# ywyue/AGILE3D

Hardware: AMD Instinct MI355X
Metric: scenes/s (80k-voxel, 10 clicks) (higher is better)
Workload: dtype f32; 1 GPU; batch of 16 synthetic 79736-voxel scenes, 10 clicks each (5 objects x 2), scene build + forward_backbone + 1 forward_mask per scene, fp32, eval; voxels=79736, queries=20, parallelism=scene-sharded x1 (no data-path collective), global_batch=16, steps_in_flight_per_gpu=4

## Files before the change

agile3d_amd/csrc/decoder.hip:

```cpp
#include "common.h"
#include <algorithm>
#include <type_traits>
#include <vector>

namespace a3d {

typedef float f32x4 __attribute__((ext_vector_type(4)));
#define A3D_GLOBAL __attribute__((address_space(1)))
template <typename T>
__device__ __forceinline__ T gld(const T* p) { return *(const T A3D_GLOBAL*)p; }
template <typename T>
__device__ __forceinline__ void gst(T* p, T v) { *(T A3D_GLOBAL*)p = v; }
__device__ __forceinline__ f32x4 gld4(const float* p) { return *(const f32x4 A3D_GLOBAL*)p; }
__device__ __forceinline__ void gst4(float* p, f32x4 v) { *(f32x4 A3D_GLOBAL*)p = v; }
__device__ __forceinline__ bool block_any(int pred, int* slot) {
  if (threadIdx.x == 0) *slot = 0;
  __syncthreads();
  if (pred) *slot = 1;
  __syncthreads();
  return *(volatile int*)slot != 0;
}
template <typename T>
__device__ __forceinline__ T gld_agent(const T* p) {
  return __hip_atomic_load((const T A3D_GLOBAL*)p, __ATOMIC_RELAXED, __HIP_MEMORY_SCOPE_AGENT);
// ... 255 lines not shown
        const bool blocked = pr >= n || (qmask[qt] && lab != obj[qt]);
        s[t] = blocked ? kNegBig : s[t];
        mx = fmaxf(mx, s[t]);
      }
      mx = rows_max(mx);
      const float mnew = fmaxf(m[qt], mx);
      const float sc = exp2_fast(m[qt] - mnew);
      m[qt] = mnew;
      f32x4 p;
      float ps = 0.f;
#pragma unroll
      for (int t = 0; t < 4; ++t) {
        p[t] = exp2_fast(s[t] - mnew);
        ps += p[t];
      }
      l[qt] = l[qt] * sc + ps;
      acc[qt] *= sc;
#pragma unroll
      for (int t = 0; t < 4; ++t) acc[qt] = __builtin_amdgcn_mfma_f32_16x16x4f32(vf[t], p[t], acc[qt], 0, 0, 0);
    }
  }
#pragma unroll
  for (int qt = 0; qt < QT; ++qt) {
    if (qt >= nqt) break;
    float lt = l[qt];
    lt = rows_sum(lt);
    float* pq = part + (((size_t)h * qp_total + qb0 + qt * 16 + j) * nchunk + chunk) * kPartStride;
    if (g == 0) {
      pq[0] = m[qt];
      pq[1] = lt;
    }
#pragma unroll
    for (int t = 0; t < 4; ++t) pq[2 + 4 * g + t] = acc[qt][t];
  }
}

template <int QT>
__global__ void __launch_bounds__(512) k_c2s_attn(const float* __restrict__ Kc, const float* __restrict__ V,
                                                  int n, const float* qproj, const int* qobj,
                                                  const unsigned char* labels, const int* counts,
                                                  float* part, int qp_total) {
  c2s_attn_body<QT>(Kc, V, n, qproj, qobj, labels, counts, part, qp_total, (int)blockIdx.y * (QT * 16), QT, (int)blockIdx.x,
                    (int)gridDim.x);
}
template <int QT>
__global__ void __launch_bounds__(512) k_c2s_attn_b(const DecSampleDev* __restrict__ samples) {
  const DecSampleDev& sm = samples[blockIdx.y];
  const int nchunk = (sm.n + kC2SChunk - 1) / kC2SChunk;
  if ((int)blockIdx.x >= nchunk) return;
  c2s_attn_body<QT>(sm.k0, sm.v0, sm.n, sm.qproj, sm.qobj, nullptr, nullptr, sm.part, sm.qp, 0, min(sm.nqt, QT), (int)blockIdx.x, nchunk);
}


template <int QT>
__global__ void __launch_bounds__(512) k_kv_c2s(const DecSampleDev* __restrict__ samples, int ns, int layer,
                                                const float* __restrict__ Wk, const float* __restrict__ Wv,
                                                const float* __restrict__ bk, const float* __restrict__ bv) {
  extern __shared__ __attribute__((aligned(16))) char smem[];
  constexpr int QP = QT * 16;
  constexpr int HW = QT <= 2 ? 4 : 2, WPG = H / HW, SPW = 8 / WPG;
  constexpr bool SWZ = QT == 4;
  constexpr int LDQ = SWZ ? 128 : 132;
  const DecSampleDev& sm = sample_of_wg(samples, ns);
  const int lb = blockIdx.x - sm.wg_begin, nwg = sm.wg_end - sm.wg_begin;
  const int n = sm.n, ngroups = (n + 15) / 16, qp_total = QP;
  const float* __restrict__ X = layer_input(sm, layer);
  const float* __restrict__ Pe = sm.posenc;
  const float* qproj = sm.qproj;
  const int* qobj = sm.qobj;
  const unsigned char* labels = layer > 0 ? sm.labels : nullptr;
  const int* counts = layer > 0 ? sm.counts + (size_t)(layer - 1) * (A3D_MAX_QUERIES + 1) : nullptr;
  float* part = sm.part;
  f32x4* Wkl = (f32x4*)smem;
  f32x4* Wvl = Wkl + 8 * 8 * 64;
  float* qp_l = (float*)(Wvl + 8 * 8 * 64);
  float* bk_l = qp_l + QP * LDQ;
  float* bv_l = bk_l + D;
  const int lane = threadIdx.x & 63, wave = threadIdx.x >> 6;
  const int g = lane >> 4, j = lane & 15;
  const int slot = lb * SPW + wave / WPG, nslots = nwg * SPW;
  f32x4 xs[8], pe[8];
  unsigned lab_nx = 0u;
  if (slot < ngroups) {
    const size_t row = (size_t)min(slot * 16 + j, n - 1);
    if (labels) lab_nx = gld((const unsigned*)(labels + slot * 16 + 4 * g));
#pragma unroll
    for (int S = 0; S < 8; ++S) xs[S] = gld4(X + row * D + 16 * S + 4 * g);
#pragma unroll
    for (int S = 0; S < 8; ++S) pe[S] = gld4(Pe + row * D + 16 * S + 4 * g);
  }
  {
    constexpr int TOT = 2 * 8 * 8 * 64;
    for (int base = threadIdx.x; base < TOT; base += 8 * 512) {
      f32x4 t8[8];
#pragma unroll
      for (int u = 0; u < 8; ++u) {
        const int e = base + u * 512;
        if (e < TOT) t8[u] = e < TOT / 2 ? ((const f32x4*)Wk)[e] : ((const f32x4*)Wv)[e - TOT / 2];
      }
#pragma unroll
      for (int u = 0; u < 8; ++u)
        if (base + u * 512 < TOT) Wkl[base + u * 512] = t8[u];
    }
  }
  for (int e = threadIdx.x; e < QP * 32; e += 512) {
    const int r = e >> 5, c = e & 31;
    *(f32x4*)(qp_l + r * LDQ + (SWZ ? (c ^ (r & 15)) : c) * 4) = gld4(qproj + (size_t)r * D + c * 4);
  }
  if (!SWZ && threadIdx.x < D) {
    bk_l[threadIdx.x] = bk[threadIdx.x];
    bv_l[threadIdx.x] = bv[threadIdx.x];
  }
  int obj[QT];
  bool qmask[QT];
#pragma unroll
  for (int qt = 0; qt < QT; ++qt) {
    obj[qt] = gld(qobj + qt * 16 + j);
    qmask[qt] = labels != nullptr && obj[qt] >= 0 && gld(counts + obj[qt]) > 0;
  }
  __syncthreads();
  const int h0 = (wave % WPG) * HW;
  f32x4 bkr[HW];
  float bvr[HW];
#pragma unroll
  for (int hl = 0; hl < HW; ++hl) {
    bkr[hl] = (f32x4){0.f, 0.f, 0.f, 0.f};
    bvr[hl] = 0.f;
    if constexpr (SWZ) {
      bkr[hl] = *(const f32x4*)(bk + 16 * (h0 + hl) + 4 * g);
      bvr[hl] = bv[16 * (h0 + hl) + j];
    }
  }
  float m[HW][QT], l[HW][QT];
  f32x4 acc[HW][QT];
#pragma unroll
  for (int hl = 0; hl < HW; ++hl)
#pragma unroll
    for (int qt = 0; qt < QT; ++qt) {
      m[hl][qt] = kNegBig;
      l[hl][qt] = 0.f;
      acc[hl][qt] = (f32x4){0.f, 0.f, 0.f, 0.f};
    }
  for (int grp = slot; grp < ngroups; grp += nslots) {
    const int p0 = grp * 16;
    const unsigned lab4 = lab_nx;
    const int next = grp + nslots < ngroups ? grp + nslots : grp;
    const size_t nrow = (size_t)min(next * 16 + j, n - 1);
    if (labels) lab_nx = gld((const unsigned*)(labels + next * 16 + 4 * g));
    f32x4 kf[HW], vv[HW];
#pragma unroll
    for (int hl = 0; hl < HW; ++hl) {
      kf[hl] = SWZ ? bkr[hl] : *(const f32x4*)(bk_l + 16 * (h0 + hl) + 4 * g);
      const float bvj = SWZ ? bvr[hl] : bv_l[16 * (h0 + hl) + j];
      vv[hl] = (f32x4){bvj, bvj, bvj, bvj};
    }
    {
      f32x4 wk = Wkl[(0 * 8 + h0) * 64 + lane], wv = Wvl[(0 * 8 + h0) * 64 + lane];
#pragma unroll
      for (int S = 0; S < 8; ++S) {
        const f32x4 xp = xs[S] + pe[S];
#pragma unroll
        for (int hl = 0; hl < HW; ++hl) {
          const int i2 = S * HW + hl + 1, S2 = i2 / HW, hl2 = i2 % HW;
          f32x4 nk = wk, nv = wv;
          if (i2 < 8 * HW) {
            nk = Wkl[(S2 * 8 + h0 + hl2) * 64 + lane];
            nv = Wvl[(S2 * 8 + h0 + hl2) * 64 + lane];
          }
          __builtin_amdgcn_sched_barrier(0);
#pragma unroll
          for (int t = 0; t < 4; ++t) {
            kf[hl] = __builtin_amdgcn_mfma_f32_16x16x4f32(wk[t], xp[t], kf[hl], 0, 0, 0);
            vv[hl] = __builtin_amdgcn_mfma_f32_16x16x4f32(xs[S][t], wv[t], vv[hl], 0, 0, 0);
          }
          __builtin_amdgcn_sched_barrier(0);
          wk = nk;
          wv = nv;
        }
        xs[S] = gld4(X + nrow * D + 16 * S + 4 * g);
        pe[S] = gld4(Pe + nrow * D + 16 * S + 4 * g);
        __builtin_amdgcn_sched_barrier(0);
      }
    }
    auto qfrag = [&](int qt, int h) {
      const int c = 4 * h + g;
      return *(const f32x4*)(qp_l + (qt * 16 + j) * LDQ + (SWZ ? (c ^ j) : c) * 4);
    };
    f32x4 qf_n = qfrag(0, h0);
    f32x4 mb[QT];
#pragma unroll
    for (int qt = 0; qt < QT; ++qt)
#pragma unroll
      for (int t = 0; t < 4; ++t) {
        const int pr = p0 + 4 * g + t;
        const int lab = (int)((lab4 >> (8 * t)) & 0xffu);
        const bool blocked = pr >= n || (qmask[qt] && lab != obj[qt]);
        mb[qt][t] = blocked ? kNegBig : 0.f;
      }
#pragma unroll
    for (int hl = 0; hl < HW; ++hl) {
      const int h = h0 + hl;
#pragma unroll
      for (int qt = 0; qt < QT; ++qt) {
        const f32x4 qf = qf_n;
        {
          const int i2 = hl * QT + qt + 1;
          if (i2 < HW * QT) qf_n = qfrag(i2 % QT, h0 + i2 / QT);
        }
        f32x4 sc4 = mb[qt];
#pragma unroll
        for (int t = 0; t < 4; ++t) sc4 = __builtin_amdgcn_mfma_f32_16x16x4f32(kf[hl][t], qf[t], sc4, 0, 0, 0);
        float mx = kNegBig;
#pragma unroll
        for (int t = 0; t < 4; ++t) mx = fmaxf(mx, sc4[t]);
        mx = rows_max(mx);
        const float mnew = fmaxf(m[hl][qt], mx);
        const float scl = exp2_fast(m[hl][qt] - mnew);
        m[hl][qt] = mnew;
        f32x4 pw;
        float ps = 0.f;
#pragma unroll
        for (int t = 0; t < 4; ++t) {
          pw[t] = exp2_fast(sc4[t] - mnew);
          ps += pw[t];
        }
        l[hl][qt] = l[hl][qt] * scl + ps;
        acc[hl][qt] *= scl;
#pragma unroll
        for (int t = 0; t < 4; ++t) acc[hl][qt] = __builtin_amdgcn_mfma_f32_16x16x4f32(vv[hl][t], pw[t], acc[hl][qt], 0, 0, 0);
      }
    }
  }
  {
    constexpr int REC = 6 * 64;
    float* red = (float*)smem;
    const int sg = wave / WPG, wl = wave % WPG;
    __syncthreads();
    if (sg > 0) {
#pragma unroll
      for (int hl = 0; hl < HW; ++hl)
#pragma unroll
        for (int qt = 0; qt < QT; ++qt) {
          float* r = red + ((size_t)((sg - 1) * WPG + wl) * (HW * QT) + hl * QT + qt) * REC + lane;
          r[0] = m[hl][qt];
          r[64] = l[hl][qt];
#pragma unroll
          for (int t = 0; t < 4; ++t) r[128 + 64 * t] = acc[hl][qt][t];
        }
    }
    __syncthreads();
    if (sg > 0) return;
#pragma unroll
    for (int hl = 0; hl < HW; ++hl)
#pragma unroll
      for (int qt = 0; qt < QT; ++qt) {
        float mm = m[hl][qt], ll = l[hl][qt];
        f32x4 aa = acc[hl][qt];
#pragma unroll
        for (int o = 1; o < SPW; ++o) {
          const float* r = red + ((size_t)((o - 1) * WPG + wl) * (HW * QT) + hl * QT + qt) * REC + lane;
          const float mo = r[0];
          const float mnew = fmaxf(mm, mo);
          const float sa = exp2_fast(mm - mnew), sb = exp2_fast(mo - mnew);
          mm = mnew;
          ll = ll * sa + r[64] * sb;
#pragma unroll
          for (int t = 0; t < 4; ++t) aa[t] = aa[t] * sa + r[128 + 64 * t] * sb;
        }
        const int h = h0 + hl;
        const float lt = rows_sum(ll);
        float* pq = part + (((size_t)h * qp_total + qt * 16 + j) * nwg + lb) * kPartStride;
        if (g == 0) {
          gst(pq, mm);
          gst(pq + 1, lt);
        }
#pragma unroll
        for (int t = 0; t < 4; ++t) gst(pq + 2 + 4 * g + t, aa[t]);
      }
  }
}
constexpr int kFusedC2SGrid = 256;

__global__ void __launch_bounds__(64) k_c2s_combine(const QuerySample* __restrict__ qs, int cached0) {
  const QuerySample& smp = qs[blockIdx.y];
  const int QP = smp.qp;
  const int q = blockIdx.x / H, h = blockIdx.x % H, lane = threadIdx.x;
  if (q >= smp.meta->nq) return;
  const float* __restrict__ part = smp.part;
  const int nchunk = cached0 ? smp.n_part0 : smp.n_part;
  float* attn = smp.B.attn;
  float m = kNegBig, l = 0.f, o[DH];
#pragma unroll
  for (int d = 0; d < DH; ++d) o[d] = 0.f;
  for (int ch = lane; ch < nchunk; ch += 64) {
    const float* p = part + (((size_t)h * QP + q) * nchunk + ch) * kPartStride;
    const float pm = gld(p);
    const float mn = fmaxf(m, pm);
    const float a = exp2f(m - mn), b = exp2f(pm - mn);
    l = l * a + gld(p + 1) * b;
#pragma unroll
    for (int d = 0; d < DH; ++d) o[d] = o[d] * a + gld(p + 2 + d) * b;
    m = mn;
  }
  float M = m;
#pragma unroll
  for (int off = 32; off > 0; off >>= 1) M = fmaxf(M, __shfl_xor(M, off, 64));
  const float sc = exp2f(m - M);
  l *= sc;
#pragma unroll
  for (int off = 32; off > 0; off >>= 1) l += __shfl_xor(l, off, 64);
#pragma unroll
  for (int d = 0; d < DH; ++d) {
    float v = o[d] * sc;
#pragma unroll
    for (int off = 32; off > 0; off >>= 1) v += __shfl_xor(v, off, 64);
    if (lane == d) gst(attn + (size_t)q * D + h * DH + d, v / l);
  }
}

template <int QT>
__global__ void __launch_bounds__(512) k_s2c_attn_wide(const float* __restrict__ Qs, int n, const float* ks,
                                                       const float* vs, int nq, int nblk, float* O) {
  constexpr int QP = QT * 16, LD = 132;
  extern __shared__ __attribute__((aligned(16))) char smem[];
// ... 411 lines not shown
      const f32x4 be = *(const f32x4*)(be_l + 16 * ct + 4 * g);
#pragma unroll
      for (int t = 0; t < 4; ++t) y[ct][t] = (y[ct][t] - mean) * rstd * ga[t] + be[t];
      if (p0 + j < n) gst4(yrow + 16 * ct + 4 * g, y[ct]);
    }
#pragma unroll
    for (int qt = 0; qt < QT; ++qt) {
      f32x4 acc = (f32x4){0.f, 0.f, 0.f, 0.f};
#pragma unroll
      for (int S = 0; S < 8; ++S) {
        const f32x4 ef = *(const f32x4*)(E_l + (qt * 16 + j) * LD + 16 * S + 4 * g);
#pragma unroll
        for (int t = 0; t < 4; ++t) acc = __builtin_amdgcn_mfma_f32_16x16x4f32(y[S][t], ef[t], acc, 0, 0, 0);
      }
#pragma unroll
      for (int t = 0; t < 4; ++t) Lw[(4 * g + t) * LL + qt * 16 + j] = acc[t];
    }
    asm volatile("s_waitcnt lgkmcnt(0)" ::: "memory");
    for (int o = g; o <= K; o += 4) {
      const int qb = o == 0 ? n_fg : qr_l[o], qe = o == 0 ? nq : qr_l[o + 1];
      float mxv = -3.4e38f;
      for (int q = qb; q < qe; ++q) mxv = fmaxf(mxv, Lw[j * LL + q]);
      Ow[j * (K + 1) + o] = mxv;
    }
    asm volatile("s_waitcnt lgkmcnt(0)" ::: "memory");
    if (lane < 16 && p0 + lane < n) {
      float best = Ow[lane * (K + 1)];
      int bi = 0;
      for (int o = 1; o <= K; ++o) {
        const float v = Ow[lane * (K + 1) + o];
        if (v > best) {
          best = v;
          bi = o;
        }
      }
      gst(labels + p0 + lane, (unsigned char)bi);
      atomicAdd(&hist[bi], 1);
    }
    const int rows = min(16, n - p0);
    for (int e = lane; e < rows * (K + 1); e += 64) gst(logits + (size_t)p0 * (K + 1) + e, Ow[e]);
    asm volatile("s_waitcnt lgkmcnt(0)" ::: "memory");
    grp = next;
  }
  __syncthreads();
  for (int e = threadIdx.x; e <= K; e += 512)
    if (hist[e]) atomicAdd(&counts[e], hist[e]);
}

template <int QT, int NW, bool KG = false, bool QC = false>
__global__ void __launch_bounds__(NW * 64) k_s2c_out(const DecSampleDev* __restrict__ samples, int ns, int layer,
                                                 const float* __restrict__ Wq, const float* __restrict__ bq,
                                                 const float* __restrict__ Wo, const float* __restrict__ bo,
                                                 const float* __restrict__ gamma, const float* __restrict__ beta, int nqr_max,
                                                 int Kmax) {
  constexpr int LD = 136, NT = NW * 64;
  constexpr bool PF = NW == 8;
  const DecSampleDev& sm = sample_of_wg(samples, ns);
  const int lb = blockIdx.x - sm.wg_begin, nwg = sm.wg_end - sm.wg_begin;
  const int n = sm.n, ngroups = (n + 15) / 16, nq = sm.nq, n_fg = sm.n_fg, K = sm.K;
  const float* __restrict__ X = layer_input(sm, layer);
  const float* __restrict__ Pe = sm.posenc;
  float* __restrict__ Y = (layer & 1) ? sm.bufD : sm.bufC;
  float* logits = sm.logits + (size_t)layer * n * (K + 1);
  unsigned char* labels = sm.labels;
  int* counts = sm.counts + (size_t)layer * (A3D_MAX_QUERIES + 1);
  const int LT = nqr_max + 4;
  extern __shared__ __attribute__((aligned(16))) char smem[];
  f32x4* Wql = (f32x4*)smem;
  f32x4* Wol = Wql + 8 * 8 * 64;
  float* ks_l = (float*)(Wol + 8 * 8 * 64);
  float* vt_l = ks_l + (KG ? 0 : nqr_max * LD);
  float* bq_l = vt_l + D * LT;
  float* bo_l = bq_l + D;
  float* ga_l = bo_l + D;
  float* be_l = ga_l + D;
  float* O_l = be_l + D;
  int* hist = (int*)(O_l + NW * 16 * (Kmax + 1));
  int* qr_l = hist + Kmax + 1;
  float* sb_l = (float*)(qr_l + Kmax + 2);
  for (int e = threadIdx.x; e < QT * 16; e += NT) sb_l[e] = e < nq ? 0.f : kNegBig;
  for (int e = threadIdx.x; e <= K + 1; e += NT) qr_l[e] = gld(sm.qrange + e);
  for (int e = threadIdx.x; e <= K; e += NT) hist[e] = 0;
  if (threadIdx.x < D) {
    bq_l[threadIdx.x] = bq[threadIdx.x];
    bo_l[threadIdx.x] = bo[threadIdx.x];
    ga_l[threadIdx.x] = gamma[threadIdx.x];
    be_l[threadIdx.x] = beta[threadIdx.x];
  }
  {
    constexpr int TOT = 8 * 8 * 64;
    for (int base = threadIdx.x; base < TOT; base += 4 * NT) {
      f32x4 t8[8];
#pragma unroll
      for (int u = 0; u < 4; ++u)
        if (base + u * NT < TOT) {
          t8[u] = ((const f32x4*)Wq)[base + u * NT];
          t8[4 + u] = ((const f32x4*)Wo)[base + u * NT];
        }
#pragma unroll
      for (int u = 0; u < 4; ++u)
        if (base + u * NT < TOT) {
          Wql[base + u * NT] = t8[u];
          Wol[base + u * NT] = t8[4 + u];
        }
    }
  }
  for (int e = threadIdx.x; e < nqr_max * 32; e += NT) {
// ... 150 lines not shown
#pragma unroll
          for (int u = 0; u < 2; ++u) vf[u][kt] = lds4((u ? vt_a1 : vt_a) + kt * 64);
#pragma unroll
        for (int kt = 0; kt < QT; ++kt)
#pragma unroll
          for (int t = 0; t < 4; ++t)
#pragma unroll
            for (int u = 0; u < 2; ++u) acc[u] = __builtin_amdgcn_mfma_f32_16x16x4f32(vf[u][kt][t], sc[u][kt][t], acc[u], 0, 0, 0);
      }
#pragma unroll
      for (int u = 0; u < 2; ++u) acc[u] *= inv[u];
#pragma unroll
      for (int i = 0; i < 8; ++i) {
        const int u = i >> 2, ct = 2 * (i & 3);
        f32x4 n0 = wo0, n1 = wo1;
        if (i + 1 < 8) {
          const int u2 = (i + 1) >> 2, ct2 = 2 * ((i + 1) & 3);
          n0 = lds4(wo_a + (u2 * 512 + ct2 * 64) * 16);
          n1 = lds4(wo_a + (u2 * 512 + ct2 * 64 + 64) * 16);
        }
        __builtin_amdgcn_sched_barrier(0);
#pragma unroll
        for (int t = 0; t < 4; ++t) {
          y[ct] = __builtin_amdgcn_mfma_f32_16x16x4f32(wo0[t], acc[u][t], y[ct], 0, 0, 0);
          y[ct + 1] = __builtin_amdgcn_mfma_f32_16x16x4f32(wo1[t], acc[u][t], y[ct + 1], 0, 0, 0);
        }
        __builtin_amdgcn_sched_barrier(0);
        wo0 = n0;
        wo1 = n1;
      }
    }
    float sum = 0.f;
#pragma unroll
    for (int ct = 0; ct < 8; ++ct) sum += y[ct][0] + y[ct][1] + y[ct][2] + y[ct][3];
    sum = rows_sum(sum);
    const float mean = sum * (1.f / D);
    float var = 0.f;
#pragma unroll
    for (int ct = 0; ct < 8; ++ct)
#pragma unroll
      for (int t = 0; t < 4; ++t) {
        const float d = y[ct][t] - mean;
        var += d * d;
      }
    var = rows_sum(var);
    const float rstd = rsqrtf(var * (1.f / D) + kLnEps);
    float* yrow = Y + (size_t)prow * D;
#pragma unroll
    for (int ct = 0; ct < 8; ++ct) {
      const f32x4 ga = *(const f32x4*)(ga_l + 16 * ct + 4 * g);
      const f32x4 be = *(const f32x4*)(be_l + 16 * ct + 4 * g);
#pragma unroll
      for (int t = 0; t < 4; ++t) y[ct][t] = (y[ct][t] - mean) * rstd * ga[t] + be[t];
      if (p0 + j < n) gst4(yrow + 16 * ct + 4 * g, y[ct]);
    }
    f32x4 ef[QT][8];
#pragma unroll
    for (int qt = 0; qt < QT; ++qt) {
      const float* er = sm.E + (size_t)min(qt * 16 + j, nq - 1) * D + 4 * g;
#pragma unroll
      for (int S = 0; S < 8; ++S) ef[qt][S] = gld4(er + 16 * S);
    }
    f32x4 lg[QT], lg2[QT];
#pragma unroll
    for (int qt = 0; qt < QT; ++qt) lg[qt] = lg2[qt] = (f32x4){0.f, 0.f, 0.f, 0.f};
#pragma unroll
    for (int S = 0; S < 8; S += 2)
#pragma unroll
      for (int t = 0; t < 4; ++t)
#pragma unroll
        for (int qt = 0; qt < QT; ++qt) {
          lg[qt] = __builtin_amdgcn_mfma_f32_16x16x4f32(ef[qt][S][t], y[S][t], lg[qt], 0, 0, 0);
          lg2[qt] = __builtin_amdgcn_mfma_f32_16x16x4f32(ef[qt][S + 1][t], y[S + 1][t], lg2[qt], 0, 0, 0);
        }
#pragma unroll
    for (int qt = 0; qt < QT; ++qt) lg[qt] += lg2[qt];
    float best = 0.f;
    int bi = 0;
    for (int o = 0; o <= K; ++o) {
      float mxv = -3.4e38f;
#pragma unroll
      for (int qt = 0; qt < QT; ++qt)
#pragma unroll
        for (int t = 0; t < 4; ++t)
          if (((oidp[qt] >> (8 * t)) & 255u) == (unsigned)o) mxv = fmaxf(mxv, lg[qt][t]);
      mxv = rows_max(mxv);
      if (g == (o & 3)) Ow[j * (K + 1) + o] = mxv;
      if (o == 0 || mxv > best) {
        best = mxv;
        bi = o;
      }
    }
    if (g == 0 && p0 + j < n) {
      gst(labels + p0 + j, (unsigned char)bi);
      atomicAdd(&hist[bi], 1);
    }
    asm volatile("s_waitcnt lgkmcnt(0)" ::: "memory");
    const int rows = min(16, n - p0);
    for (int e = lane; e < rows * (K + 1); e += 64) gst(logits + (size_t)p0 * (K + 1) + e, Ow[e]);
    asm volatile("s_waitcnt lgkmcnt(0)" ::: "memory");
    grp = next;
  }
  __syncthreads();
  for (int e = threadIdx.x; e <= K; e += NT)
    if (hist[e]) atomicAdd(&counts[e], hist[e]);
}

struct QueryLayerW {
  const float *c2s_in_wt, *c2s_in_b, *c2s_out_wt, *c2s_out_b, *c2s_norm_w, *c2s_norm_b;
  const float *c2c_in_wt, *c2c_in_b, *c2c_out_wt, *c2c_out_b, *c2c_norm_w, *c2c_norm_b;
  const float *ffn_w1t, *ffn_b1, *ffn_w2t, *ffn_b2, *ffn_norm_w, *ffn_norm_b;
  const float *s2c_in_wt, *s2c_in_b;
  const float *dn_w, *dn_b, *m_w0t, *m_b0, *m_w2t, *m_b2;
  const float *next_c2s_in_wt, *next_c2s_in_b;
  const float *qpack, *next_qpack, *mpack;
  int dim_ff;
  int layer;
};


constexpr int kLinKC = 256, kLinLD = kLinKC + 4;
template <int QT>
__device__ __noinline__ void lin(const float* X, int ldx, const float* Xadd, int Q, int K, const float* __restrict__ W,
                                 int ldw, const float* __restrict__ bias, int N, float* Y, int ldy, bool relu,
                                 float scale, float* lds ) {
  const int tid = threadIdx.x, nt = blockDim.x;
  const int lane = tid & 63, wave = tid >> 6, nw = nt >> 6;
  const int g = lane >> 4, j = lane & 15;
  const int ntiles = N >> 4;
  for (int t0 = 0; t0 < ntiles; t0 += nw) {
    const int ntile = t0 + wave;
    const bool active = ntile < ntiles;
    f32x4 acc[QT];
#pragma unroll
    for (int qt = 0; qt < QT; ++qt) acc[qt] = (f32x4){0.f, 0.f, 0.f, 0.f};
    for (int kc = 0; kc < K; kc += kLinKC) {
      const int kcur = min(kLinKC, K - kc);
      __syncthreads();
      for (int e = tid; e < QT * 16 * (kcur >> 2); e += nt) {
        const int q = e / (kcur >> 2), k4 = (e - q * (kcur >> 2)) * 4;
        f32x4 v = (f32x4){0.f, 0.f, 0.f, 0.f};
        if (q < Q) {
          v = gld4(X + (size_t)q * ldx + kc + k4);
          if (Xadd) v += gld4(Xadd + (size_t)q * D + kc + k4);
        }
        *(f32x4*)(lds + q * kLinLD + k4) = v;
      }
      __syncthreads();
      if (active) {
        const float* wrow = W + (size_t)(ntile * 16 + j) * ldw + kc + 4 * g;
#pragma unroll 4
        for (int S = 0; S < (kcur >> 4); ++S) {
          const f32x4 b = gld4(wrow + 16 * S);
#pragma unroll
          for (int qt = 0; qt < QT; ++qt) {
// ... 794 lines not shown
    k_pack_rows<<<(unsigned)((n4 + 255) / 256), 256, 0, st>>>(W, N, K, out_dev + off);
  };
  if (layer < 0) {
    if (!w->mask_w0 || !w->mask_w2) {
      set_error("a3d_decoder_pack_query_weights: mask head weights missing");
      return A3D_ERR_INVALID;
    }
    pack(w->mask_w0, D, D, kMpW0);
    pack(w->mask_w2, D, D, kMpW2);
  } else {
    const a3d_decoder_layer& LW = w->layers[layer];
    if (!LW.c2s_out_w || !LW.c2c_in_w || !LW.c2c_out_w || !LW.s2c_in_w || !LW.c2s_in_w || !LW.ffn_w1 || !LW.ffn_w2) {
      set_error("a3d_decoder_pack_query_weights: layer %d weights missing", layer);
      return A3D_ERR_INVALID;
    }
    pack(LW.c2s_out_w, D, D, kQpC2sOut);
    pack(LW.c2c_in_w, 3 * D, D, kQpC2cIn);
    pack(LW.c2c_out_w, D, D, kQpC2cOut);
    pack(LW.s2c_in_w + (size_t)D * D, 2 * D, D, kQpS2cKV);
    pack(LW.c2s_in_w, D, D, kQpC2sQ);
    pack(LW.ffn_w1, w->dim_ff, D, kQpFfn1);
    pack(LW.ffn_w2, D, w->dim_ff, qpack_ffn2(w->dim_ff));
  }
  A3D_LAUNCH_CHECK();
  return A3D_OK;
}

static bool fused_c2s() {
  static int v = -1;
  if (v < 0) {
    const char* e = getenv("A3D_FUSED_C2S");
    v = e ? atoi(e) : 1;
  }
  return v != 0;
}

static bool fused_wide() {
  static int v = -1;
  if (v < 0) {
    const char* e = getenv("A3D_FUSED_WIDE");
    v = e ? atoi(e) : 1;
  }
  return v != 0 && fused_c2s();
}

static bool fused_s2o() {
  static int v = -1;
  if (v < 0) {
    const char* e = getenv("A3D_FUSED_S2O");
    v = e ? atoi(e) : 1;
  }
  return v != 0;
}
static int wide_from() {
  static int v = -1;
  if (v < 0) {
    const char* e = getenv("A3D_WIDE_FROM");
    v = e ? atoi(e) : 33;
    v = v < 17 ? 17 : v;
  }
  return v;
}

struct Prepared {
  QueryMeta hm;
  DecLayout L;
  char* ws;
  const float *feats, *posenc;
  int n;
  float* logits;
  float* kv0 = nullptr;
  int kv0_state = 0;
  int qtw = 0;
  float *bufA, *bufB, *bufC, *bufD, *part;
  unsigned char* labels;
  int* counts;
  QueryMeta* meta;
  QueryBufs B;
  int wg_begin, wg_end;
  void bind() {
    bufA = (float*)(ws + L.buf[0]);
    bufB = (float*)(ws + L.buf[1]);
    bufC = (float*)(ws + L.buf[2]);
    bufD = (float*)(ws + L.buf[3]);
    labels = (unsigned char*)(ws + L.labels);
    counts = (int*)(ws + L.counts);
    part = (float*)(ws + L.part);
    meta = (QueryMeta*)(ws + L.meta);
    B.queries = (float*)(ws + L.q[0]);
    B.qpos = (float*)(ws + L.q[1]);
    B.qproj = (float*)(ws + L.q[2]);
    B.ks = (float*)(ws + L.q[3]);
    B.vs = (float*)(ws + L.q[4]);
    B.E = (float*)(ws + L.q[5]);
    B.attn = (float*)(ws + L.q[6]);
    B.tmp = (float*)(ws + L.q[7]);
    B.tgt = (float*)(ws + L.q[8]);
    B.qk = (float*)(ws + L.q[9]);
    B.vc = (float*)(ws + L.q[10]);
    B.hidden = (float*)(ws + L.q[11]);
  }
};

struct DecTables {
  int grid;
  DecSampleDev* samples_dev;
// ... 114 lines not shown
    if (nblk == 1) {
      k_query_block<QT, 0><<<dim3(nh_env, 1, ns), 512, qb_lds, st>>>(qs_dev, QW);
    } else if constexpr (QT == 4 || QT == 2) {
      k_query_block<QT, 1><<<dim3(1, nblk, ns), 512, qb_lds, st>>>(qs_dev, QW);
      k_query_block<QT, 2><<<dim3(nh_env, nblk, ns), 512, qb_lds, st>>>(qs_dev, QW);
    }
  }
  A3D_LAUNCH_CHECK();
  return A3D_OK;
}

template <int QT>
static int run_decoder(const a3d_decoder_weights* w, Prepared* P, int ns, hipStream_t st) {
  constexpr int QP = QT * 16;
  const int nblk = P[0].L.qp / QP;
  {
    static bool big = false;
    if (!big) {
      big = true;
      const int big_lds = 160 * 1024;
      A3D_ALLOW_LDS(big_lds, k_query_block<1, 0>);
      A3D_ALLOW_LDS(big_lds, k_query_block<2, 0>);
      A3D_ALLOW_LDS(big_lds, k_query_block<3, 0>);
      A3D_ALLOW_LDS(big_lds, k_query_block<4, 0>);
      A3D_ALLOW_LDS(big_lds, k_query_block<4, 1>);
      A3D_ALLOW_LDS(big_lds, k_query_block<4, 2>);
      A3D_ALLOW_LDS(big_lds, k_s2c_attn_wide<4>);
      A3D_ALLOW_LDS(big_lds, k_q_s2c<1>);
      A3D_ALLOW_LDS(big_lds, k_q_s2c<2>);
      A3D_ALLOW_LDS(big_lds, k_q_s2c<3>);
      A3D_ALLOW_LDS(big_lds, k_q_s2c<4>);
      A3D_ALLOW_LDS(big_lds, k_out_ln_mask<1>);
      A3D_ALLOW_LDS(big_lds, k_out_ln_mask<2>);
      A3D_ALLOW_LDS(big_lds, k_out_ln_mask<3>);
      A3D_ALLOW_LDS(big_lds, k_out_ln_mask<4>);
      A3D_ALLOW_LDS(big_lds, k_s2c_out<1, 8>);
      A3D_ALLOW_LDS(big_lds, k_s2c_out<2, 8>);
      A3D_ALLOW_LDS(big_lds, k_s2c_out<1, 12>);
      A3D_ALLOW_LDS(big_lds, k_s2c_out<2, 12>);
      A3D_ALLOW_LDS(big_lds, (k_s2c_out<2, 12, true>));
      A3D_ALLOW_LDS(big_lds, (k_s2c_out<2, 8, true>));
      A3D_ALLOW_LDS(big_lds, (k_s2c_out<1, 12, true>));
      A3D_ALLOW_LDS(big_lds, (k_s2c_out<1, 8, true>));
      A3D_ALLOW_LDS(big_lds, (k_q_s2c<1, true>));
      A3D_ALLOW_LDS(big_lds, (k_q_s2c<2, true>));
      A3D_ALLOW_LDS(big_lds, (k_q_s2c<3, true>));
      A3D_ALLOW_LDS(big_lds, (k_q_s2c<4, true>));
      A3D_ALLOW_LDS(big_lds, (k_s2c_out<1, 12, false, true>));
      A3D_ALLOW_LDS(big_lds, (k_s2c_out<2, 12, false, true>));
      A3D_ALLOW_LDS(big_lds, (k_s2c_out<1, 12, true, true>));
      A3D_ALLOW_LDS(big_lds, (k_s2c_out<2, 12, true, true>));
      A3D_ALLOW_LDS(big_lds, k_kv_c2s<1>);
      A3D_ALLOW_LDS(big_lds, k_kv_c2s<2>);
      A3D_ALLOW_LDS(big_lds, k_kv_c2s<3>);
      A3D_ALLOW_LDS(big_lds, k_kv_c2s<4>);
      A3D_ALLOW_LDS(big_lds, k_ln_mask<4>);
    }
  }
  const int n_counts = A3D_MAX_DEC_LAYERS * (A3D_MAX_QUERIES + 1);
  int64_t n_total = 0;
  int Kmax = 0, nq_max = 0;
  for (int si = 0; si < ns; ++si) {
    Prepared& p = P[si];
    n_total += p.n;
    Kmax = p.hm.K > Kmax ? p.hm.K : Kmax;
    nq_max = p.hm.nq > nq_max ? p.hm.nq : nq_max;
  }
  const size_t s2c_lds = (size_t)2 * QP * 132 * 4;
  const size_t qs2c_lds = ((size_t)QP * 132 + (size_t)D * (QP + 4) + D) * 4;
  const size_t fused_lds = (size_t)64 * 1024 + ((size_t)3 * D + QP * 132 + 8 * 16 * (QP + 1) + 8 * 16 * (Kmax + 1)) * 4 +
                           (size_t)(2 * Kmax + 3) * 4;
  for (int si = 0; si < ns; ++si) {
    const size_t lnm_lds = ((size_t)QP * 132 + 4 * 16 * (P[si].L.qp + 1) + 4 * 16 * (P[si].hm.K + 1)) * 4 + (size_t)(P[si].hm.K + 1) * 4;
    if (lnm_lds > 160 * 1024) {
      set_error("a3d_decoder_forward: %d queries x %d objects need %zu bytes of LDS in the mask head", P[si].hm.nq,
                P[si].hm.K, lnm_lds);
      return A3D_ERR_UNSUPPORTED;
    }
  }
  const bool fuse_c2s = fused_c2s() && nblk == 1;
  const bool fuse_s2c = fused_c2s() && nblk == 1;
  const bool fuse_out = fuse_s2c && fused_lds <= 160 * 1024;
  const int nqr_max = (nq_max + 3) & ~3;
  const size_t s2c_rest = ((size_t)D * (nqr_max + 4) + 4 * D + (size_t)8 * 16 * (Kmax + 1) + 2 * Kmax + 3 + QT * 16 + 1) * 4;
  const size_t s2c_keys = (size_t)nqr_max * 136 * 4;
  const size_t staging12 = (size_t)4 * 16 * (Kmax + 1) * 4;
  const bool s2c_kg = (size_t)128 * 1024 + s2c_keys + s2c_rest + staging12 > 160 * 1024;
  const size_t s2c_out_lds = (size_t)128 * 1024 + (s2c_kg ? 0 : s2c_keys) + s2c_rest;
  const size_t s2c_out_lds12 = s2c_out_lds + staging12;
  static int fused_s2c_env = -1;
  if (fused_s2c_env < 0) {
    const char* e = getenv("A3D_FUSED_S2C");
    fused_s2c_env = e ? atoi(e) : 1;
  }
  const bool fuse_all = fuse_out && fused_s2c_env && QT <= 2 && s2c_out_lds <= 160 * 1024;
  DecTables T;
  {
    const int rc_t = upload_tables(P, ns, false, fuse_c2s, st, T);
    if (rc_t) return rc_t;
  }
  const int grid = T.grid;
  DecSampleDev* const samples_dev = T.samples_dev;
  QuerySample* const qs_dev = T.qs_dev;
  {
    ProfScope ps(st, A3D_PROF_QUERY, 0, 0, 0, 0, nq_max);
    k_query_init<QT><<<dim3(nblk, ns), 512, 0, st>>>(qs_dev, w->bg_query_feat, w->bg_query_pos, w->time_table,
                                                    w->layers[0].c2s_in_w, w->layers[0].c2s_in_b, n_counts);
    A3D_LAUNCH_CHECK();
  }
  for (int l = 0; l < w->n_layers; ++l) {
    const a3d_decoder_layer& LW = w->layers[l];
    int rc;
    bool cached0 = l == 0;
    for (int si = 0; si < ns && cached0; ++si) cached0 = P[si].kv0 != nullptr && P[si].kv0_state != 0;
    const bool qc0 = cached0;
    if (cached0) {
      for (int si = 0; si < ns; ++si) {
        Prepared& p = P[si];
        float* K0 = p.kv0;
        float* V0 = p.kv0 + (size_t)p.n * D;
        if (p.kv0_state == 1) {
          rc = a3d_linear(p.feats, D, p.posenc, D, p.n, D, D, LW.c2s_wk_packed, nullptr, LW.c2s_in_b + D, nullptr, 0, 0, K0, D, nullptr, 0, st);
          if (rc) return rc;
          rc = a3d_linear(p.feats, D, nullptr, 0, p.n, D, D, LW.c2s_wv_packed, nullptr, LW.c2s_in_b + 2 * D, nullptr, 0, 0, V0, D, nullptr, 0, st);
          if (rc) return rc;
          rc = a3d_linear(p.feats, D, p.posenc, D, p.n, D, D, LW.s2c_wq_packed, nullptr, LW.s2c_in_b, nullptr, 0, 0,
                          p.kv0 + (size_t)2 * p.n * D, D, nullptr, 0, st);
          if (rc) return rc;
        }
        if (nblk == 1) continue;
        ProfScope ps(st, A3D_PROF_C2S, 0, 0, 0, 0, p.n);
        k_c2s_attn<QT><<<dim3(p.L.nchunk, nblk), 512, 0, st>>>(K0, V0, p.n, p.B.qproj, p.meta->obj, nullptr, nullptr, p.part, p.L.qp);
        A3D_LAUNCH_CHECK();
      }
      if (nblk == 1) {
        int nchunk_max = 0;
        for (int si = 0; si < ns; ++si) nchunk_max = P[si].L.nchunk > nchunk_max ? P[si].L.nchunk : nchunk_max;
        ProfScope ps(st, A3D_PROF_C2S, 0, 0, 0, 0, (int)n_total);
        k_c2s_attn_b<QT><<<dim3(nchunk_max, ns), 512, 0, st>>>(samples_dev);
        A3D_LAUNCH_CHECK();
      }
    } else if (fuse_c2s) {
      ProfScope ps(st, A3D_PROF_C2S, 0, 0, 0, 0, (int)n_total);
      const size_t c2s_lds = (size_t)128 * 1024 + (QT == 4 ? (size_t)QP * 128 * 4 : ((size_t)QP * 132 + 2 * D) * 4);
      k_kv_c2s<QT><<<grid, 512, c2s_lds, st>>>(samples_dev, ns, l, LW.c2s_wk_packed, LW.c2s_wv_packed, LW.c2s_in_b + D,
                                               LW.c2s_in_b + 2 * D);
      A3D_LAUNCH_CHECK();
    } else {
      for (int si = 0; si < ns; ++si) {
        Prepared& p = P[si];
        const float* src = l == 0 ? p.feats : (((l - 1) & 1) ? p.bufD : p.bufC);
        const int* prev_counts = l > 0 ? p.counts + (size_t)(l - 1) * (A3D_MAX_QUERIES + 1) : nullptr;
        rc = a3d_linear(src, D, p.posenc, D, p.n, D, D, LW.c2s_wk_packed, nullptr, LW.c2s_in_b + D, nullptr, 0, 0, p.bufA, D, nullptr, 0, st);
        if (rc) return rc;
        rc = a3d_linear(src, D, nullptr, 0, p.n, D, D, LW.c2s_wv_packed, nullptr, LW.c2s_in_b + 2 * D, nullptr, 0, 0, p.bufB, D, nullptr, 0, st);
        if (rc) return rc;
        ProfScope ps(st, A3D_PROF_C2S, 0, 0, 0, 0, p.n);
        k_c2s_attn<QT><<<dim3(p.L.nchunk, nblk), 512, 0, st>>>(p.bufA, p.bufB, p.n, p.B.qproj, p.meta->obj,
                                                              l > 0 ? p.labels : nullptr, prev_counts, p.part, p.L.qp);
        A3D_LAUNCH_CHECK();
      }
    }
    rc = launch_query_side<QT>(w, l, qs_dev, P[0].L.qp, nblk, ns, nq_max, cached0, st);
    if (rc) return rc;
    if (fuse_all) {
      ProfScope ps(st, A3D_PROF_S2C, 0, 0, 0, 0, (int)n_total);
      if constexpr (QT <= 2) {
        if (qc0 && s2c_kg && s2c_out_lds12 <= 160 * 1024)
          k_s2c_out<QT, 12, true, true><<<grid, 768, s2c_out_lds12, st>>>(samples_dev, ns, l, LW.s2c_wq_packed, LW.s2c_in_b, LW.s2c_wo_packed,
                                                                         LW.s2c_out_b, LW.s2c_norm_w, LW.s2c_norm_b, nqr_max, Kmax);
        else if (qc0 && !s2c_kg && s2c_out_lds12 <= 160 * 1024)
          k_s2c_out<QT, 12, false, true><<<grid, 768, s2c_out_lds12, st>>>(samples_dev, ns, l, LW.s2c_wq_packed, LW.s2c_in_b, LW.s2c_wo_packed,
                                                                          LW.s2c_out_b, LW.s2c_norm_w, LW.s2c_norm_b, nqr_max, Kmax);
        else if (s2c_kg && s2c_out_lds12 <= 160 * 1024)
          k_s2c_out<QT, 12, true><<<grid, 768, s2c_out_lds12, st>>>(samples_dev, ns, l, LW.s2c_wq_packed, LW.s2c_in_b, LW.s2c_wo_packed,
                                                                   LW.s2c_out_b, LW.s2c_norm_w, LW.s2c_norm_b, nqr_max, Kmax);
        else if (s2c_kg)
          k_s2c_out<QT, 8, true><<<grid, 512, s2c_out_lds, st>>>(samples_dev, ns, l, LW.s2c_wq_packed, LW.s2c_in_b, LW.s2c_wo_packed,
                                                                LW.s2c_out_b, LW.s2c_norm_w, LW.s2c_norm_b, nqr_max, Kmax);
        else if (s2c_out_lds12 <= 160 * 1024)
          k_s2c_out<QT, 12><<<grid, 768, s2c_out_lds12, st>>>(samples_dev, ns, l, LW.s2c_wq_packed, LW.s2c_in_b, LW.s2c_wo_packed,
                                                             LW.s2c_out_b, LW.s2c_norm_w, LW.s2c_norm_b, nqr_max, Kmax);
        else
          k_s2c_out<QT, 8><<<grid, 512, s2c_out_lds, st>>>(samples_dev, ns, l, LW.s2c_wq_packed, LW.s2c_in_b, LW.s2c_wo_packed,
                                                          LW.s2c_out_b, LW.s2c_norm_w, LW.s2c_norm_b, nqr_max, Kmax);
      }
      A3D_LAUNCH_CHECK();
      continue;
    }
    if (fuse_s2c) {
      ProfScope ps(st, A3D_PROF_S2C, 0, 0, 0, 0, (int)n_total);
      if (qc0) k_q_s2c<QT, true><<<grid, 512, (size_t)64 * 1024 + qs2c_lds, st>>>(samples_dev, ns, l, LW.s2c_wq_packed, LW.s2c_in_b);
      else k_q_s2c<QT><<<grid, 512, (size_t)64 * 1024 + qs2c_lds, st>>>(samples_dev, ns, l, LW.s2c_wq_packed, LW.s2c_in_b);
      A3D_LAUNCH_CHECK();
    } else {
      for (int si = 0; si < ns; ++si) {
        Prepared& p = P[si];
        const float* src = l == 0 ? p.feats : (((l - 1) & 1) ? p.bufD : p.bufC);
        const float* Qs = p.bufA;
        if (qc0) {
          Qs = p.kv0 + (size_t)2 * p.n * D;
        } else {
          rc = a3d_linear(src, D, p.posenc, D, p.n, D, D, LW.s2c_wq_packed, nullptr, LW.s2c_in_b, nullptr, 0, 0, p.bufA, D, nullptr, 0, st);
          if (rc) return rc;
        }
        ProfScope ps(st, A3D_PROF_S2C, 0, 0, 0, 0, p.n);
        k_s2c_attn_wide<QT><<<(p.n + 127) / 128, 512, s2c_lds, st>>>(Qs, p.n, p.B.ks, p.B.vs, p.hm.nq, nblk, p.bufB);
        A3D_LAUNCH_CHECK();
      }
    }
    if (fuse_out) {
      ProfScope ps(st, A3D_PROF_LNMASK, 0, 0, 0, 0, (int)n_total);
      k_out_ln_mask<QT><<<grid, 512, fused_lds, st>>>(samples_dev, ns, l, LW.s2c_wo_packed, LW.s2c_out_b, LW.s2c_norm_w,
                                                      LW.s2c_norm_b);
      A3D_LAUNCH_CHECK();
    } else {
      for (int si = 0; si < ns; ++si) {
        Prepared& p = P[si];
        const float* src = l == 0 ? p.feats : (((l - 1) & 1) ? p.bufD : p.bufC);
        float* Y = (l & 1) ? p.bufD : p.bufC;
        const int K = p.hm.K;
        const size_t lnm_lds = ((size_t)QP * 132 + 4 * 16 * (p.L.qp + 1) + 4 * 16 * (K + 1)) * 4 + (size_t)(K + 1) * 4;
        rc = a3d_linear(p.bufB, D, nullptr, 0, p.n, D, D, LW.s2c_wo_packed, nullptr, LW.s2c_out_b, src, D, 0, Y, D, nullptr, 0, st);
        if (rc) return rc;
        ProfScope ps(st, A3D_PROF_LNMASK, 0, 0, 0, 0, p.n);
        k_ln_mask<QT><<<(p.n + 63) / 64, 256, lnm_lds, st>>>(Y, p.n, LW.s2c_norm_w, LW.s2c_norm_b, p.B.E, p.hm.nq, p.meta->qrange,
                                                          p.hm.n_fg, K, p.logits + (size_t)l * p.n * (K + 1), p.labels,
                                                          p.counts + (size_t)l * (A3D_MAX_QUERIES + 1), nblk);
        A3D_LAUNCH_CHECK();
      }
    }
  }
  return A3D_OK;
}

template <int QT>
static int run_decoder_wide(const a3d_decoder_weights* w, Prepared* P, int ns, hipStream_t st) {
  int qp = 0;
// ... 353 lines not shown
```

Baseline: 639.6 scenes/s.

## Pack leftover 17–20 query tile into block-diagonal MFMA in fused c2s attention

For 20 queries with QT=2, the second 16-query tile holds only 4 real queries. The kernel now builds a block-diagonal packed query matrix in LDS, so one MFMA chain per head group scores the 4 leftover queries across all 4 heads at once, and a single softmax update covers them. This cuts the redundant second-tile MFMA and exp work, but adds extra LDS and a new partial-write layout. Separately, the last decoder layer's s2c output kernel skips writing features, labels and histograms that no later layer reads.

```diff
diff --git a/agile3d_amd/csrc/decoder.hip b/agile3d_amd/csrc/decoder.hip
--- a/agile3d_amd/csrc/decoder.hip
+++ b/agile3d_amd/csrc/decoder.hip
@@ -331,10 +331,12 @@
 }
 
 
-template <int QT>
+constexpr int kQdLD = 20;
+template <int QT, bool PK = false>
 __global__ void __launch_bounds__(512) k_kv_c2s(const DecSampleDev* __restrict__ samples, int ns, int layer,
                                                 const float* __restrict__ Wk, const float* __restrict__ Wv,
                                                 const float* __restrict__ bk, const float* __restrict__ bv) {
+  static_assert(!PK || QT == 2, "the packed leftover tile is the 17..20-query build");
   extern __shared__ __attribute__((aligned(16))) char smem[];
   constexpr int QP = QT * 16;
   constexpr int HW = QT <= 2 ? 4 : 2, WPG = H / HW, SPW = 8 / WPG;
@@ -355,9 +357,11 @@
   float* qp_l = (float*)(Wvl + 8 * 8 * 64);
   float* bk_l = qp_l + QP * LDQ;
   float* bv_l = bk_l + D;
+  float* qd_l = bv_l + D;
   const int lane = threadIdx.x & 63, wave = threadIdx.x >> 6;
   const int g = lane >> 4, j = lane & 15;
   const int slot = lb * SPW + wave / WPG, nslots = nwg * SPW;
+  constexpr bool packed = PK;
   f32x4 xs[8], pe[8];
   unsigned lab_nx = 0u;
   if (slot < ngroups) {
@@ -390,11 +394,19 @@
     bk_l[threadIdx.x] = bk[threadIdx.x];
     bv_l[threadIdx.x] = bv[threadIdx.x];
   }
+  if constexpr (PK) {
+    {
+      const int h = threadIdx.x >> 6, c = (threadIdx.x >> 2) & 15, c4 = threadIdx.x & 3;
+      f32x4 v = (f32x4){0.f, 0.f, 0.f, 0.f};
+      if ((c >> 2) == (h & 3)) v = gld4(qproj + (size_t)(16 + (c & 3)) * D + 16 * h + 4 * c4);
+      *(f32x4*)(qd_l + (h * 16 + c) * kQdLD + 4 * c4) = v;
+    }
+  }
   int obj[QT];
   bool qmask[QT];
 #pragma unroll
   for (int qt = 0; qt < QT; ++qt) {
-    obj[qt] = gld(qobj + qt * 16 + j);
+    obj[qt] = gld(qobj + (qt == 1 && packed ? 16 + (j & 3) : qt * 16 + j));
     qmask[qt] = labels != nullptr && obj[qt] >= 0 && gld(counts + obj[qt]) > 0;
   }
   __syncthreads();
@@ -420,6 +432,8 @@
       l[hl][qt] = 0.f;
       acc[hl][qt] = (f32x4){0.f, 0.f, 0.f, 0.f};
     }
+  unsigned qd_a = PK ? (unsigned)(size_t)qd_l + (unsigned)((h0 * 16 + j) * kQdLD + 4 * g) * 4u : 0u;
+  if constexpr (PK) asm volatile("" : "+v"(qd_a));
   for (int grp = slot; grp < ngroups; grp += nslots) {
     const int p0 = grp * 16;
     const unsigned lab4 = lab_nx;
@@ -476,6 +490,61 @@
         const bool blocked = pr >= n || (qmask[qt] && lab != obj[qt]);
         mb[qt][t] = blocked ? kNegBig : 0.f;
       }
+    if constexpr (PK) {
+      {
+        f32x4 scp = mb[1];
+#pragma unroll
+        for (int hl = 0; hl < HW; ++hl) {
+          const f32x4 qf = hl == 0 ? qf_n : qfrag(0, h0 + hl);
+          const f32x4 qd = *(const __attribute__((address_space(3))) f32x4*)(qd_a + hl * 16 * kQdLD * 4);
+          f32x4 sc4 = mb[0];
+#pragma unroll
+          for (int t = 0; t < 4; ++t) sc4 = __builtin_amdgcn_mfma_f32_16x16x4f32(kf[hl][t], qf[t], sc4, 0, 0, 0);
+#pragma unroll
+          for (int t = 0; t < 4; ++t) scp = __builtin_amdgcn_mfma_f32_16x16x4f32(kf[hl][t], qd[t], scp, 0, 0, 0);
+          float mx = kNegBig;
+#pragma unroll
+          for (int t = 0; t < 4; ++t) mx = fmaxf(mx, sc4[t]);
+          mx = rows_max(mx);
+          const float mnew = fmaxf(m[hl][0], mx);
+          const float scl = exp2_fast(m[hl][0] - mnew);
+          m[hl][0] = mnew;
+          f32x4 pw;
+          float ps = 0.f;
+#pragma unroll
+          for (int t = 0; t < 4; ++t) {
+            pw[t] = exp2_fast(sc4[t] - mnew);
+            ps += pw[t];
+          }
+          l[hl][0] = l[hl][0] * scl + ps;
+          acc[hl][0] *= scl;
+#pragma unroll
+          for (int t = 0; t < 4; ++t) acc[hl][0] = __builtin_amdgcn_mfma_f32_16x16x4f32(vv[hl][t], pw[t], acc[hl][0], 0, 0, 0);
+        }
+        float mx = kNegBig;
+#pragma unroll
+        for (int t = 0; t < 4; ++t) mx = fmaxf(mx, scp[t]);
+        mx = rows_max(mx);
+        const float mnew = fmaxf(m[0][1], mx);
+        const float scl = exp2_fast(m[0][1] - mnew);
+        m[0][1] = mnew;
+        f32x4 pw;
+        float ps = 0.f;
+#pragma unroll
+        for (int t = 0; t < 4; ++t) {
+          pw[t] = exp2_fast(scp[t] - mnew);
+          ps += pw[t];
+        }
+        l[0][1] = l[0][1] * scl + ps;
+#pragma unroll
+        for (int hl = 0; hl < HW; ++hl) acc[hl][1] *= scl;
+#pragma unroll
+        for (int t = 0; t < 4; ++t)
+#pragma unroll
+          for (int hl = 0; hl < HW; ++hl) acc[hl][1] = __builtin_amdgcn_mfma_f32_16x16x4f32(vv[hl][t], pw[t], acc[hl][1], 0, 0, 0);
+        continue;
+      }
+    }
 #pragma unroll
     for (int hl = 0; hl < HW; ++hl) {
       const int h = h0 + hl;
@@ -514,6 +583,15 @@
     constexpr int REC = 6 * 64;
     float* red = (float*)smem;
     const int sg = wave / WPG, wl = wave % WPG;
+    if constexpr (PK) {
+      {
+#pragma unroll
+        for (int hl = 1; hl < HW; ++hl) {
+          m[hl][1] = m[0][1];
+          l[hl][1] = l[0][1];
+        }
+      }
+    }
     __syncthreads();
     if (sg > 0) {
 #pragma unroll
@@ -548,7 +626,9 @@
         }
         const int h = h0 + hl;
         const float lt = rows_sum(ll);
-        float* pq = part + (((size_t)h * qp_total + qt * 16 + j) * nwg + lb) * kPartStride;
+        const bool pk = qt == 1 && packed;
+        if (pk && (j >> 2) != hl) continue;
+        float* pq = part + (((size_t)h * qp_total + (pk ? 16 + (j & 3) : qt * 16 + j)) * nwg + lb) * kPartStride;
         if (g == 0) {
           gst(pq, mm);
           gst(pq + 1, lt);
@@ -1066,7 +1146,7 @@
                                                  const float* __restrict__ Wq, const float* __restrict__ bq,
                                                  const float* __restrict__ Wo, const float* __restrict__ bo,
                                                  const float* __restrict__ gamma, const float* __restrict__ beta, int nqr_max,
-                                                 int Kmax) {
+                                                 int Kmax, int last) {
   constexpr int LD = 136, NT = NW * 64;
   constexpr bool PF = NW == 8;
   const DecSampleDev& sm = sample_of_wg(samples, ns);
@@ -1323,7 +1403,7 @@
       const f32x4 be = *(const f32x4*)(be_l + 16 * ct + 4 * g);
 #pragma unroll
       for (int t = 0; t < 4; ++t) y[ct][t] = (y[ct][t] - mean) * rstd * ga[t] + be[t];
-      if (p0 + j < n) gst4(yrow + 16 * ct + 4 * g, y[ct]);
+      if (!last && p0 + j < n) gst4(yrow + 16 * ct + 4 * g, y[ct]);
     }
     f32x4 ef[QT][8];
 #pragma unroll
@@ -1362,7 +1442,7 @@
         bi = o;
       }
     }
-    if (g == 0 && p0 + j < n) {
+    if (!last && g == 0 && p0 + j < n) {
       gst(labels + p0 + j, (unsigned char)bi);
       atomicAdd(&hist[bi], 1);
     }
@@ -1372,6 +1452,7 @@
     asm volatile("s_waitcnt lgkmcnt(0)" ::: "memory");
     grp = next;
   }
+  if (last) return;
   __syncthreads();
   for (int e = threadIdx.x; e <= K; e += NT)
     if (hist[e]) atomicAdd(&counts[e], hist[e]);
@@ -2272,6 +2353,15 @@
   }
   return v != 0;
 }
+static bool pack_tile() {
+  static int v = -1;
+  if (v < 0) {
+    const char* e = getenv("A3D_PACK_TILE");
+    v = e ? (atoi(e) != 0) : 1;
+  }
+  return v != 0;
+}
+
 static int wide_from() {
   static int v = -1;
   if (v < 0) {
@@ -2492,6 +2582,7 @@
       A3D_ALLOW_LDS(big_lds, (k_s2c_out<2, 12, true, true>));
       A3D_ALLOW_LDS(big_lds, k_kv_c2s<1>);
       A3D_ALLOW_LDS(big_lds, k_kv_c2s<2>);
+      A3D_ALLOW_LDS(big_lds, (k_kv_c2s<2, true>));
       A3D_ALLOW_LDS(big_lds, k_kv_c2s<3>);
       A3D_ALLOW_LDS(big_lds, k_kv_c2s<4>);
       A3D_ALLOW_LDS(big_lds, k_ln_mask<4>);
@@ -2519,6 +2610,8 @@
     }
   }
   const bool fuse_c2s = fused_c2s() && nblk == 1;
+  bool pack_c2s = QT == 2 && pack_tile();
+  for (int si = 0; si < ns; ++si) pack_c2s = pack_c2s && P[si].hm.nq > 16 && P[si].hm.nq <= 20;
   const bool fuse_s2c = fused_c2s() && nblk == 1;
   const bool fuse_out = fuse_s2c && fused_lds <= 160 * 1024;
   const int nqr_max = (nq_max + 3) & ~3;
@@ -2582,9 +2675,16 @@
       }
     } else if (fuse_c2s) {
       ProfScope ps(st, A3D_PROF_C2S, 0, 0, 0, 0, (int)n_total);
-      const size_t c2s_lds = (size_t)128 * 1024 + (QT == 4 ? (size_t)QP * 128 * 4 : ((size_t)QP * 132 + 2 * D) * 4);
-      k_kv_c2s<QT><<<grid, 512, c2s_lds, st>>>(samples_dev, ns, l, LW.c2s_wk_packed, LW.c2s_wv_packed, LW.c2s_in_b + D,
-                                               LW.c2s_in_b + 2 * D);
+      const size_t c2s_lds = (size_t)128 * 1024 + (QT == 4 ? (size_t)QP * 128 * 4 : ((size_t)QP * 132 + 2 * D) * 4) +
+                             (pack_c2s ? (size_t)H * 16 * kQdLD * 4 : 0);
+      if constexpr (QT == 2) {
+        if (pack_c2s)
+          k_kv_c2s<2, true><<<grid, 512, c2s_lds, st>>>(samples_dev, ns, l, LW.c2s_wk_packed, LW.c2s_wv_packed, LW.c2s_in_b + D,
+                                                        LW.c2s_in_b + 2 * D);
+      }
+      if (!pack_c2s)
+        k_kv_c2s<QT><<<grid, 512, c2s_lds, st>>>(samples_dev, ns, l, LW.c2s_wk_packed, LW.c2s_wv_packed, LW.c2s_in_b + D,
+                                                 LW.c2s_in_b + 2 * D);
       A3D_LAUNCH_CHECK();
     } else {
       for (int si = 0; si < ns; ++si) {
@@ -2605,25 +2705,26 @@
     if (rc) return rc;
     if (fuse_all) {
       ProfScope ps(st, A3D_PROF_S2C, 0, 0, 0, 0, (int)n_total);
+      const int last = l == w->n_layers - 1 ? 1 : 0;
       if constexpr (QT <= 2) {
         if (qc0 && s2c_kg && s2c_out_lds12 <= 160 * 1024)
           k_s2c_out<QT, 12, true, true><<<grid, 768, s2c_out_lds12, st>>>(samples_dev, ns, l, LW.s2c_wq_packed, LW.s2c_in_b, LW.s2c_wo_packed,
-                                                                         LW.s2c_out_b, LW.s2c_norm_w, LW.s2c_norm_b, nqr_max, Kmax);
+                                                                         LW.s2c_out_b, LW.s2c_norm_w, LW.s2c_norm_b, nqr_max, Kmax, last);
         else if (qc0 && !s2c_kg && s2c_out_lds12 <= 160 * 1024)
           k_s2c_out<QT, 12, false, true><<<grid, 768, s2c_out_lds12, st>>>(samples_dev, ns, l, LW.s2c_wq_packed, LW.s2c_in_b, LW.s2c_wo_packed,
-                                                                          LW.s2c_out_b, LW.s2c_norm_w, LW.s2c_norm_b, nqr_max, Kmax);
+                                                                          LW.s2c_out_b, LW.s2c_norm_w, LW.s2c_norm_b, nqr_max, Kmax, last);
         else if (s2c_kg && s2c_out_lds12 <= 160 * 1024)
           k_s2c_out<QT, 12, true><<<grid, 768, s2c_out_lds12, st>>>(samples_dev, ns, l, LW.s2c_wq_packed, LW.s2c_in_b, LW.s2c_wo_packed,
-                                                                   LW.s2c_out_b, LW.s2c_norm_w, LW.s2c_norm_b, nqr_max, Kmax);
+                                                                   LW.s2c_out_b, LW.s2c_norm_w, LW.s2c_norm_b, nqr_max, Kmax, last);
         else if (s2c_kg)
           k_s2c_out<QT, 8, true><<<grid, 512, s2c_out_lds, st>>>(samples_dev, ns, l, LW.s2c_wq_packed, LW.s2c_in_b, LW.s2c_wo_packed,
-                                                                LW.s2c_out_b, LW.s2c_norm_w, LW.s2c_norm_b, nqr_max, Kmax);
+                                                                LW.s2c_out_b, LW.s2c_norm_w, LW.s2c_norm_b, nqr_max, Kmax, last);
         else if (s2c_out_lds12 <= 160 * 1024)
           k_s2c_out<QT, 12><<<grid, 768, s2c_out_lds12, st>>>(samples_dev, ns, l, LW.s2c_wq_packed, LW.s2c_in_b, LW.s2c_wo_packed,
-                                                             LW.s2c_out_b, LW.s2c_norm_w, LW.s2c_norm_b, nqr_max, Kmax);
+                                                             LW.s2c_out_b, LW.s2c_norm_w, LW.s2c_norm_b, nqr_max, Kmax, last);
         else
           k_s2c_out<QT, 8><<<grid, 512, s2c_out_lds, st>>>(samples_dev, ns, l, LW.s2c_wq_packed, LW.s2c_in_b, LW.s2c_wo_packed,
-                                                          LW.s2c_out_b, LW.s2c_norm_w, LW.s2c_norm_b, nqr_max, Kmax);
+                                                          LW.s2c_out_b, LW.s2c_norm_w, LW.s2c_norm_b, nqr_max, Kmax, last);
       }
       A3D_LAUNCH_CHECK();
       continue;
```

Measured after the change: 641.3 scenes/s, median of 4. About the same (+0.3%).
